# christianhbye/21cmVAE

Hardware: AMD Instinct MI355X
Metric: emulated signals/sec (batched predict) (higher is better)
Workload: dtype f16 (f32 accumulate)

## Files before the change

21cmvae_amd/csrc/api_forward.hip:

```cpp
#include "api_internal.h"

namespace v21 {
#define V21_DECL(a)                                                      \
  hipError_t launch_fused_##a##_F32(const FusedArgs&, hipStream_t);      \
  hipError_t launch_fused_##a##_F16x2sp(const FusedArgs&, hipStream_t);  \
  hipError_t launch_fused_##a##_BF16x2sp(const FusedArgs&, hipStream_t);
V21_ARCH_LIST(V21_DECL)
#undef V21_DECL
hipError_t launch_fused_S1_F16x2spClk(const FusedArgs&, hipStream_t);
hipError_t launch_fused_S1_BF16x2spClk(const FusedArgs&, hipStream_t);
}

typedef hipError_t (*fused_launcher)(const FusedArgs&, hipStream_t);
struct FusedEntry {
  int L;
  const int* dims;
  const int* act;
  fused_launcher fn[3];
};
#define V21_ENTRY(a) \
  {Arch##a::L, Arch##a::dims, Arch##a::act, {launch_fused_##a##_F32, launch_fused_##a##_F16x2sp, launch_fused_##a##_BF16x2sp}},
static const FusedEntry g_fused[] = {V21_ARCH_LIST(V21_ENTRY)};
#undef V21_ENTRY


static int fpi_of(int prec) { return prec == V21_PREC_F32 ? 8 : 16; }
static void stream_geometry(const v21_mlp* m, int prec, int* total, int* padded) {
  int f = 0;
  for (int l = 0; l < m->L; ++l) f += ((m->dims[l + 1] + 31) / 32) * ((m->dims[l] + fpi_of(prec) - 1) / fpi_of(prec) + 1);
  *total = f;
  *padded = (f + 7) / 8 * 8;
}

static int fused_id_of(int n_layers, const int* dims, const int* act) {
  for (size_t i = 0; i < sizeof(g_fused) / sizeof(g_fused[0]); ++i) {
    const FusedEntry& fe = g_fused[i];
    if (fe.L != n_layers) continue;
    bool same = true;
    for (int k = 0; k <= n_layers && same; ++k) same = fe.dims[k] == dims[k];
    for (int k = 0; k < n_layers && same; ++k) same = fe.act[k] == act[k];
    if (same) return (int)i;
// ... 72 lines not shown
  return V21_OK;
}
extern "C" int v21_mlp_destroy(v21_mlp* m) {
  if (!m) return V21_OK;
  hipSetDevice(m->ctx->device);
  hipStreamSynchronize(m->ctx->stream);
  delete m;
  return V21_OK;
}
extern "C" int v21_mlp_num_params(const v21_mlp* m, size_t* n) {
  if (!m || !n) return fail(V21_ERR_ARG, "null argument");
  *n = m->nparams;
  return V21_OK;
}
void invalidate_streams(v21_mlp* m) {
  for (int i = 0; i < 3; ++i) m->stream_ok[i] = false;
  for (int i = 0; i < 3; ++i) m->cfw_ok[i] = false;
  m->wpad_ok = false;
  m->wt_ok = false;
}

extern "C" int v21_mlp_set_weights(v21_mlp* m, const float* flat, size_t n) {
  if (!m || !flat) return fail(V21_ERR_ARG, "null argument");
  if (n != m->nparams) return fail(V21_ERR_ARG, "set_weights: got %zu floats, stack has %zu", n, m->nparams);
  CHK(use(m->ctx));
  HIPCHK(hipMemcpyAsync(m->d_w, flat, n * sizeof(float), hipMemcpyHostToDevice, m->ctx->stream));
  HIPCHK(hipStreamSynchronize(m->ctx->stream));
  invalidate_streams(m);
  return V21_OK;
}
extern "C" int v21_mlp_get_weights(v21_mlp* m, float* flat, size_t n) {
// ... 27 lines not shown
  if (t->n != m->dims[m->L] || !t->mean) return fail(V21_ERR_ARG, "output transform: n = %d, stack output = %d", t->n, m->dims[m->L]);
  CHK(m->d_mean.reserve((size_t)t->n));
  HIPCHK(hipMemcpyAsync(m->d_mean, t->mean, (size_t)t->n * sizeof(float), hipMemcpyHostToDevice, m->ctx->stream));
  HIPCHK(hipStreamSynchronize(m->ctx->stream));
  m->out_std = t->std;
  m->has_tout = true;
  return V21_OK;
}
extern "C" int v21_mlp_has_fused(const v21_mlp* m, int precision, int* yes) {
  if (!m || !yes) return fail(V21_ERR_ARG, "null argument");
  if (precision < 0 || precision > 2) return fail(V21_ERR_ARG, "precision %d unknown", precision);
  *yes = m->fused_id >= 0 ? 1 : 0;
  return V21_OK;
}

static int ensure_stream(v21_mlp* m, int prec) {
  if (m->stream_ok[prec]) return V21_OK;
  int total, padded;
  stream_geometry(m, prec, &total, &padded);
  Dev<unsigned char>& dst = m->d_stream[prec];
  CHK(dst.reserve((size_t)padded * 1024));
  PackArgs pa{};
  pa.w = m->d_w;
  pa.mean = m->has_tout ? m->d_mean : nullptr;
  pa.stream = dst;
  pa.L = m->L;
  pa.total = total;
  pa.padded = padded;
  pa.fpi = fpi_of(prec);
  pa.epi = prec == V21_PREC_F32 ? 4 : 8;
  pa.esize = prec == V21_PREC_F32 ? 4 : 2;
  pa.is_bf16 = prec == V21_PREC_BF16;
  int f = 0;
  for (int l = 0; l < m->L; ++l) {
    PackLayer& pl = pa.lt[l];
    pl.K = m->dims[l]; pl.N = m->dims[l + 1];
    pl.ks = (pl.K + pa.fpi - 1) / pa.fpi; pl.nt = (pl.N + 31) / 32;
    pl.w_off = m->w_off[l]; pl.b_off = m->b_off[l];
    pl.first = f;
    f += pl.nt * (pl.ks + 1);
  }
  hipLaunchKernelGGL(pack_stream_kernel, dim3((padded + 3) / 4), dim3(256), 0, m->ctx->stream, pa);
  HIPCHK(hipGetLastError());
  m->stream_ok[prec] = true;
  return V21_OK;
}

int mlp_fused_stream(v21_mlp* m, int prec, const unsigned char** stream) {
  CHK(ensure_stream(m, prec));
  *stream = m->d_stream[prec];
  return V21_OK;
}

template <class P, int EP>
static int launch_gemm(GemmArgs g, hipStream_t st) {
  if (g.M <= 0 || g.N <= 0) return V21_OK;
  dim3 grid((g.N + kBN - 1) / kBN, (g.M + kBM - 1) / kBM);
  const bool akc = g.sa_k == 1, bkc = g.sb_k == 1;
  if (!akc && g.sa_m != 1) return fail(V21_ERR_ARG, "gemm: A must be contiguous along m or k");
  if (!bkc && g.sb_n != 1) return fail(V21_ERR_ARG, "gemm: B must be contiguous along k or n");
  if (akc && bkc) hipLaunchKernelGGL((gemm_kernel<P, EP, true, true>), grid, dim3(256), 0, st, g);
  else if (akc) hipLaunchKernelGGL((gemm_kernel<P, EP, true, false>), grid, dim3(256), 0, st, g);
  else if (bkc) hipLaunchKernelGGL((gemm_kernel<P, EP, false, true>), grid, dim3(256), 0, st, g);
  else hipLaunchKernelGGL((gemm_kernel<P, EP, false, false>), grid, dim3(256), 0, st, g);
  HIPCHK(hipGetLastError());
  return V21_OK;
}
// ... 102 lines not shown
      (!(flags & V21_FWD_IN_TRANSFORM) || m->dims[0] <= 8)) {
    v21::JitKernel* k = jit_kernel(m, precision);
    if (force_jit && k) v21::jit_wait(k, -1);
    if (jit_ready(k)) jk = k;
    if (force_jit && !jk) {
      std::string why = "not eligible, or V21_JIT=0";
      if (k) v21::jit_state(k, &why);
      return fail(V21_ERR_UNSUPPORTED, "V21_FWD_FORCE_JIT: no run-time kernel for this stack: %s", why.c_str());
    }
  }
  q.jit = jk ? 2 : 0;
  int route = decide_forward(q);
  FusedArgs a{};
  hipError_t rt = hipSuccess;
  if (route == FWD_FUSED || route == FWD_FUSED_RT) {
    CHK(ensure_stream(m, precision));
    a.x = d_x; a.ldx = ldx; a.y = d_y; a.ldy = ldy; a.n_rows = n;
    a.stream = m->d_stream[precision];
    const bool tout = (flags & V21_FWD_OUT_TRANSFORM) != 0;
    a.out_std = tout ? m->out_std : 1.0f;
    a.out_mean_scale = tout ? 1.0f : 0.0f;
    a.in_transform = (flags & V21_FWD_IN_TRANSFORM) ? 1 : 0;
    if (a.in_transform) a.tin = m->tin;
#ifdef V21_FUSED_STAMP
    a.dbg = (unsigned long long*)(getenv("V21_FUSED_DBG_PTR") ? strtoull(getenv("V21_FUSED_DBG_PTR"), nullptr, 0) : 0ull);
#endif
  }
  if (route == FWD_FUSED_RT) {
    rt = v21::jit_launch(jk, m->ctx->device, a, m->ctx->stream);
    if (rt != hipSuccess) (void)hipGetLastError();
    if (rt != hipSuccess && !force_jit) { q.jit = 0; route = decide_forward(q); }
  }
  note_route(m, route);
// ... 270 lines not shown
```

21cmvae_amd/csrc/api_internal.h:

```cpp
#pragma once
#include <dlfcn.h>
#include <hip/hip_runtime.h>

#include <algorithm>
#include <climits>
#include <cmath>
#include <cstdarg>
#include <cstdio>
#include <cstdlib>
#include <cstring>
#include <functional>
#include <memory>
#include <string>
#include <vector>

#pragma GCC visibility push(default)
#include "../../include/v21.h"
#pragma GCC visibility pop
#include "archs.h"
#include "fused_fwd.h"
#include "jit.h"
#include "gemm.h"
#include "gemm_nt.h"
#include "train_kernels.h"
// ... 99 lines not shown
};

struct NuisRecord {
  std::vector<double> q, r, cd;
  std::vector<float> qf, proj;
};

struct v21_mlp {
  v21_ctx* ctx = nullptr;
  int L = 0;
  std::vector<int> dims, act;
  std::vector<long long> w_off, b_off;
  size_t nparams = 0;
  Dev<float> d_w;
  int fused_id = -1;
  Dev<unsigned char> d_stream[3];
  bool stream_ok[3] = {false, false, false};
  bool has_tin = false, has_tout = false;
  v21_affine_in tin{};
  float out_std = 1.f;
  Dev<float> d_mean;
  Dev<float> d_act[2];
  Dev<float> d_xs, d_ys;
  Dev<double> d_xs64;
  int maxdim = 0;
  bool wpad_ok = false;
  Dev<float> d_wt;
  std::vector<long long> wt_off;
  bool wt_ok = false;
  Dev<float> d_small[2];
  Dev<float> d_xpad;
  Dev<unsigned char> d_cfw[3], d_cbw[3];
// ... 234 lines not shown
```

21cmvae_amd/csrc/fused_fwd.h:

```cpp
#pragma once
#ifndef __HIPCC_RTC__
#include <hip/hip_runtime.h>
#endif

#include <type_traits>
#include <utility>

#include "../../include/v21_types.h"
#include "par_transform.h"

namespace v21 {

typedef float f32x16 __attribute__((ext_vector_type(16)));
typedef float f32x4 __attribute__((ext_vector_type(4)));
typedef _Float16 f16x8 __attribute__((ext_vector_type(8)));
typedef __bf16 bf16x8 __attribute__((ext_vector_type(8)));
typedef unsigned u32x4 __attribute__((ext_vector_type(4)));
typedef short i16x2 __attribute__((ext_vector_type(2)));
typedef float f32x2 __attribute__((ext_vector_type(2)));
typedef _Float16 f16x2 __attribute__((ext_vector_type(2)));
typedef __bf16 bf16x2 __attribute__((ext_vector_type(2)));

constexpr int kFragBytes = 1024;
constexpr int kWaves = 4;
// ... 30 lines not shown
  long long n_rows;
  const unsigned char* stream;
  float out_std;
  float out_mean_scale;
  int in_transform;
  v21_affine_in tin;
  unsigned long long* dbg;
};

struct PrecF16 {
  static constexpr int BLK = 24, RING = 4, WPS = 1, DEPTH = 2, WAVES = 4;
  using frag = f16x8;
  using elem = _Float16;
  static constexpr int FPI = 16, EPI = 8, CT = 2;
  static constexpr int WPI = 4;
  static __device__ __forceinline__ unsigned pack2(float a, float b) {
    f32x2 v = {a, b};
    return __builtin_bit_cast(unsigned, __builtin_convertvector(v, f16x2));
  }
  template <bool SWAP> static __device__ __forceinline__ f32x16 mfma(frag w, frag x, f32x16 c) {
    if constexpr (!SWAP) return __builtin_amdgcn_mfma_f32_32x32x16_f16(w, x, c, 0, 0, 0);
    else return __builtin_amdgcn_mfma_f32_32x32x16_f16(x, w, c, 0, 0, 0);
  }
};
struct PrecBF16 {
  static constexpr int BLK = 24, RING = 4, WPS = 1, DEPTH = 2, WAVES = 4;
  using frag = bf16x8;
  using elem = __bf16;
  static constexpr int FPI = 16, EPI = 8, CT = 2;
  static constexpr int WPI = 4;
  static __device__ __forceinline__ unsigned pack2(float a, float b) {
    f32x2 v = {a, b};
    return __builtin_bit_cast(unsigned, __builtin_convertvector(v, bf16x2));
  }
  template <bool SWAP> static __device__ __forceinline__ f32x16 mfma(frag w, frag x, f32x16 c) {
    if constexpr (!SWAP) return __builtin_amdgcn_mfma_f32_32x32x16_bf16(w, x, c, 0, 0, 0);
    else return __builtin_amdgcn_mfma_f32_32x32x16_bf16(x, w, c, 0, 0, 0);
  }
};
struct PrecF32 {
  static constexpr int BLK = 24, RING = 4, WPS = 1, DEPTH = 2, WAVES = 4;
  using frag = f32x4;
  using elem = float;
  static constexpr int FPI = 8, EPI = 4, CT = 1;
  static constexpr int WPI = 4;
// ... 11 lines not shown
struct PrecF16x2 : PrecF16 { static constexpr int CT = 1, BLK = 16, RING = 4, WPS = 2; };
struct PrecBF16x2 : PrecBF16 { static constexpr int CT = 1, BLK = 16, RING = 4, WPS = 2; };
#else
struct PrecF16x2 : PrecF16 { static constexpr int CT = 1, BLK = 16, RING = 5, WPS = 2; };
struct PrecBF16x2 : PrecBF16 { static constexpr int CT = 1, BLK = 16, RING = 5, WPS = 2; };
#endif

struct PrecF16x2sp : PrecF16x2 { static constexpr bool SPREAD_DMA = true; };
struct PrecBF16x2sp : PrecBF16x2 { static constexpr bool SPREAD_DMA = true; };
struct PrecF16x2spClk : PrecF16x2sp { static constexpr bool CLOCK_STAMPS = true; };
struct PrecBF16x2spClk : PrecBF16x2sp { static constexpr bool CLOCK_STAMPS = true; };
template <class P, class = void> struct clk_of { static constexpr bool value = false; };
template <class P> struct clk_of<P, std::void_t<decltype(P::CLOCK_STAMPS)>> { static constexpr bool value = P::CLOCK_STAMPS; };
template <class P, class = void> struct spread_of { static constexpr bool value = false; };
template <class P> struct spread_of<P, std::void_t<decltype(P::SPREAD_DMA)>> { static constexpr bool value = P::SPREAD_DMA; };

template <class Arch, class P> struct Geo {
  static constexpr int L = Arch::L;
  static constexpr int FPI = P::FPI;
  static constexpr int BLK = P::BLK, RING = P::RING, WAVES = P::WAVES;
  static constexpr int IPT = 16 / P::EPI;
  static constexpr int dim(int i) { return Arch::dims[i]; }
  static constexpr int act(int l) { return Arch::act[l]; }
  static constexpr int ks_of(int l) { return (dim(l) + FPI - 1) / FPI; }
  static constexpr int nt_of(int l) { return (dim(l + 1) + 31) / 32; }
  static constexpr int tile_base(int l, int nt) {
    int f = 0;
    for (int i = 0; i < l; ++i) f += nt_of(i) * (ks_of(i) + 1);
    return f + nt * (ks_of(l) + 1);
  }
// ... 44 lines not shown
  static constexpr int chunks_per_kstep(int G, int nchunks) {
    const int lim = spread_limit(G);
    return lim <= 0 ? nchunks : (nchunks + lim - 1) / lim;
  }
  static constexpr int stores_before_step(int S, int CT, int D) {
    int s = 0;
    const int l = L - 1, nch = CT * 8;
    for (int nt = 0; nt + 1 < nt_of(l); ++nt) {
      const int cpk = chunks_per_kstep(gtile(l, nt), nch);
      const int nb = tile_base(l, nt + 1);
      for (int c = 0; c < nch; ++c)
        if (nb + 1 + c / cpk + D < S) s += 2;
    }
    return s;
  }
};

template <int N> __device__ __forceinline__ void wait_vmcnt_barrier() {
  static_assert(N >= 0 && N <= 63, "vmcnt is 6 bits");
  asm volatile("s_waitcnt vmcnt(%0)\n\ts_barrier" ::"n"(N) : "memory");
}

__device__ __forceinline__ void glds16(const unsigned char* sbase, unsigned voff, unsigned lds_dst) {
  asm volatile("s_mov_b32 m0, %2\n\ts_nop 0\n\tglobal_load_lds_dwordx4 %0, %1"
               :
               : "v"(voff), "s"(sbase), "s"(lds_dst)
               : "memory");
}
__device__ __forceinline__ unsigned lds_addr(const void* p) {
  return (unsigned)(unsigned long long)(const __attribute__((address_space(3))) void*)p;
// ... 16 lines not shown

template <class G, int B, int I>
__device__ __forceinline__ void issue_piece(const unsigned char* gstream, unsigned char* smem,
                                            int wave, int lane) {
  if constexpr (B >= 0 && B < G::n_blocks()) {
    if constexpr (I < G::blk_glds(B)) {
      const unsigned char* g = gstream + (size_t)B * G::BLK * kFragBytes + I * G::WAVES * kFragBytes;
      const unsigned voff = wave * kFragBytes + lane * 16;
      const unsigned s = lds_addr(smem) + (B % G::RING) * G::BLK * kFragBytes + wave * kFragBytes +
                         I * G::WAVES * kFragBytes;
      glds16(g, voff, s);
    }
  }
}

template <class G, int CT, int D, int S, bool SPREAD>
__device__ __forceinline__ void ring_boundary(const unsigned char* gstream, unsigned char* smem,
                                              int wave, int lane, unsigned long long* g_dbg = nullptr) {
  constexpr int kBlkFrags = G::BLK, kRing = G::RING;
  if constexpr (S % kBlkFrags == 0 && S < G::padded()) {
    constexpr int B = S / kBlkFrags;
    constexpr int last_issued = (B + kRing - 3 > kRing - 1) ? B + kRing - 3 : kRing - 1;
    constexpr int GA = [] {
      int s = 0;
      for (int i = B + 1; i <= last_issued; ++i) s += G::blk_glds(i);
      return s;
    }();
    constexpr int S_issue = (B < kRing) ? 0 : (B - kRing + 2 + (SPREAD ? 1 : 0)) * kBlkFrags;
    constexpr int SA = G::stores_before_step(S, CT, D) - G::stores_before_step(S_issue, CT, D);
    constexpr int N = (GA + SA) > 63 ? 63 : (GA + SA);
#ifdef V21_FUSED_STAMP
    { unsigned long long t; asm volatile("s_memtime %0\n\ts_waitcnt lgkmcnt(0)" : "=s"(t)::"memory");
      ((unsigned long long*)(smem + G::RING * G::BLK * kFragBytes))[wave * 512 + 2 * B] = t; }
#endif
    wait_vmcnt_barrier<N>();
#ifdef V21_FUSED_STAMP
    { unsigned long long t; asm volatile("s_memtime %0\n\ts_waitcnt lgkmcnt(0)" : "=s"(t)::"memory");
      ((unsigned long long*)(smem + G::RING * G::BLK * kFragBytes))[wave * 512 + 2 * B + 1] = t; }
#endif
    if constexpr (B >= 2 && !SPREAD) issue_block<G, B + kRing - 2>(gstream, smem, wave, lane);
  }
}

template <class G, int F> __device__ __forceinline__ const unsigned char* frag_ptr(const unsigned char* smem, int lane) {
  constexpr int B = F / G::BLK;
// ... 10 lines not shown
  using frag = typename P::frag;
  using Item = typename G::Item;
  constexpr int L = G::L, CT = P::CT, EPI = P::EPI, FPI = P::FPI, IPT = G::IPT;
  constexpr int KSM = G::ks_max();
#ifndef V21_FUSED_D
#define V21_FUSED_D 2
#endif
#ifndef V21_FUSED_SPREAD
#define V21_FUSED_SPREAD 0
#endif
  constexpr int D = P::DEPTH;
  constexpr bool SPREAD = (V21_FUSED_SPREAD != 0) || spread_of<P>::value;
  constexpr int TOTAL = G::total();
  constexpr int NOUT = G::dim(L);
  constexpr int NCH = CT * 8;
  static_assert(G::act(L - 1) == 0, "output layer must be linear");
  static_assert(G::nt_of(L - 1) == 1 || G::ks_of(L - 1) > P::DEPTH, "output layer: too few k-steps per tile for the aux double buffer");
  static_assert(D <= kBlkFrags, "read-ahead must stay within one block");

  const int lane = threadIdx.x & 63;
  const int wave = __builtin_amdgcn_readfirstlane(threadIdx.x >> 6);
  const int r = lane & 31, h = lane >> 5;
  unsigned long long clk_t0 = 0, clk_r0 = 0;
  if constexpr (clk_of<P>::value) {
    asm volatile("s_memtime %0\n\ts_memrealtime %1\n\ts_waitcnt lgkmcnt(0)" : "=s"(clk_t0), "=s"(clk_r0)::"memory");
  }
  const long long wg_row0 = (long long)blockIdx.x * (kWaves * CT * 32);
  const long long row0 = wg_row0 + wave * (CT * 32);

  unsigned bufA[CT][KSM][4], bufB[CT][KSM][4];
// ... 43 lines not shown
    issue_block<G, decltype(b)::value>(a.stream, smem, wave, lane);
  });

  long long wg_rows = a.n_rows - wg_row0;
  if (wg_rows > kWaves * CT * 32) wg_rows = kWaves * CT * 32;
  if (wg_rows < 0) wg_rows = 0;
  const unsigned out_bytes = (unsigned)(wg_rows * a.ldy * 4);
  __amdgpu_buffer_rsrc_t orsrc =
      __builtin_amdgcn_make_buffer_rsrc((void*)(a.y + wg_row0 * a.ldy), 0, out_bytes, 0x00020000);
  const unsigned ldy_b = (unsigned)a.ldy * 4u;
  const unsigned ovoff = (unsigned)(wave * (CT * 32) + 4 * h) * ldy_b + (unsigned)r * 4u;

  frag q[D + 1];
  f32x16 auxb[2];
  f32x16 acc[2][CT];

  auto epilogue_chunk = [&](auto g_, auto c_) __attribute__((always_inline)) {
    constexpr int GT = decltype(g_)::value;
    constexpr int c = decltype(c_)::value;
    constexpr Item t = G::tile_at(GT);
    constexpr int l = t.l, nt = t.nt;
    constexpr int ct = c / 8, pr = c % 8;
    if constexpr (l < L - 1) {
      constexpr int item = IPT * nt + (2 * pr) / EPI, e0 = (2 * pr) % EPI;
      if constexpr (item < G::ks_of(l + 1)) {
        auto& out = (l & 1) ? bufA : bufB;
        const float x0 = acc[GT & 1][ct][2 * pr], x1 = acc[GT & 1][ct][2 * pr + 1];
        if constexpr (EPI == 8) {
          unsigned w = P::pack2(x0, x1);
          if constexpr (G::act(l) != 0) {
// ... 28 lines not shown
  };
  auto epilogue_range = [&](auto g_, auto lo_, auto hi_) __attribute__((always_inline)) {
    constexpr int LO = decltype(lo_)::value, HI = decltype(hi_)::value;
    static_for<(HI > LO ? HI - LO : 0)>([&](auto k) __attribute__((always_inline)) {
      epilogue_chunk(g_, std::integral_constant<int, LO + decltype(k)::value>{});
    });
  };
  auto operand = [&](auto& buf, int ct, int ks) __attribute__((always_inline)) {
    const u32x4 wds = {buf[ct][ks][0], buf[ct][ks][1], buf[ct][ks][2], buf[ct][ks][3]};
    return __builtin_bit_cast(frag, wds);
  };

  static_for<TOTAL + D>([&](auto s_) __attribute__((always_inline)) {
    constexpr int S = decltype(s_)::value;
    if constexpr (S < TOTAL) {
      ring_boundary<G, CT, D, S, SPREAD>(a.stream, smem, wave, lane, a.dbg);
      if constexpr (SPREAD && S / kBlkFrags >= 2) {
        constexpr int Bc = S / kBlkFrags, o = S % kBlkFrags;
#ifndef V21_SP_PHASE
#define V21_SP_PHASE 3
#endif
        if constexpr (o % G::WAVES == V21_SP_PHASE % G::WAVES)
          issue_piece<G, Bc + kRing - 2, o / G::WAVES>(a.stream, smem, wave, lane);
      }
      constexpr Item it = G::item_at(S);
      if constexpr (it.ks >= 0) {
        q[S % (D + 1)] = *(const frag*)frag_ptr<G, S>(smem, lane);
      } else {
        constexpr int GT = G::gtile(it.l, it.nt);
        const unsigned char* aux = frag_ptr<G, S>(smem, 0);
        if constexpr (it.l < L - 1) {
          const f32x4* bp = (const f32x4*)(aux + h * 64);
#pragma unroll
          for (int qd = 0; qd < 4; ++qd) {
            const f32x4 t = bp[qd];
            auxb[GT & 1][4 * qd + 0] = t[0]; auxb[GT & 1][4 * qd + 1] = t[1];
            auxb[GT & 1][4 * qd + 2] = t[2]; auxb[GT & 1][4 * qd + 3] = t[3];
          }
        } else {
          auxb[GT & 1][0] = ((const float*)aux)[r];
          auxb[GT & 1][1] = ((const float*)aux)[32 + r];
        }
      }
    }
    if constexpr (S >= D) {
      constexpr int C = S - D;
      constexpr Item it = G::item_at(C);
      if constexpr (it.ks >= 0) {
        constexpr int GT = G::gtile(it.l, it.nt);
        constexpr int GP = GT > 0 ? GT - 1 : 0;
        constexpr int CPK = G::chunks_per_kstep(GP, NCH);
        constexpr bool whole_first = (GT > 0) && (G::spread_limit(GP) == 0);
        if constexpr (whole_first && it.ks == 0) {
          epilogue_range(std::integral_constant<int, GP>{}, std::integral_constant<int, 0>{},
                         std::integral_constant<int, NCH>{});
        }
#ifdef V21_FUSED_STAMP
        if constexpr (it.ks == 0) {
          unsigned long long t; asm volatile("s_memtime %0\n\ts_waitcnt lgkmcnt(0)" : "=s"(t)::"memory");
          ((unsigned long long*)(smem + kFusedLds))[wave * 512 + 128 + GT] = t; }
#endif
        auto& in = (it.l & 1) ? bufB : bufA;
        const frag w = q[C % (D + 1)];
#pragma unroll
        for (int ct = 0; ct < CT; ++ct) {
          f32x16 c0;
          if constexpr (it.ks == 0) {
            if constexpr (it.l < L - 1) c0 = auxb[GT & 1];
            else
#pragma unroll
              for (int i = 0; i < 16; ++i) c0[i] = 0.f;
          } else {
            c0 = acc[GT & 1][ct];
          }
          acc[GT & 1][ct] = P::template mfma<(it.l == L - 1)>(w, operand(in, ct, it.ks), c0);
        }
        if constexpr (GT > 0 && !whole_first) {
          constexpr int lo = it.ks * CPK < NCH ? it.ks * CPK : NCH;
          constexpr int hi = (it.ks + 1) * CPK < NCH ? (it.ks + 1) * CPK : NCH;
          epilogue_range(std::integral_constant<int, GP>{}, std::integral_constant<int, lo>{},
                         std::integral_constant<int, hi>{});
        }
      }
    }
  });
  epilogue_range(std::integral_constant<int, G::n_tiles() - 1>{}, std::integral_constant<int, 0>{},
                 std::integral_constant<int, NCH>{});
  if constexpr (clk_of<P>::value) {
    unsigned long long t1, r1;
    unsigned xcc, hwid;
    asm volatile("s_memtime %0\n\ts_memrealtime %1\n\ts_getreg_b32 %2, hwreg(HW_REG_XCC_ID)\n\ts_getreg_b32 %3, hwreg(HW_REG_HW_ID)\n\ts_waitcnt lgkmcnt(0)"
                 : "=s"(t1), "=s"(r1), "=s"(xcc), "=s"(hwid)::"memory");
    if (a.dbg && wave == 0 && lane == 0) {
      unsigned long long* gd = a.dbg + (size_t)blockIdx.x * 5;
      gd[0] = clk_t0; gd[1] = clk_r0; gd[2] = t1; gd[3] = r1; gd[4] = (unsigned long long)(xcc & 0xF) | ((unsigned long long)hwid << 8);
    }
  }
#ifdef V21_FUSED_STAMP
  if (a.dbg) {
    unsigned long long t; asm volatile("s_memtime %0\n\ts_waitcnt lgkmcnt(0)" : "=s"(t)::"memory");
    unsigned long long* sd = (unsigned long long*)(smem + kFusedLds) + wave * 512;
    sd[127] = t;
// ... 10 lines not shown
```

21cmvae_amd/csrc/jit.hip:

```cpp
#include "jit.h"
#include "fused_train16.h"

#include <dlfcn.h>
#include <signal.h>
#include <spawn.h>
#include <sys/stat.h>
#include <sys/wait.h>
#include <unistd.h>

#include <atomic>
#include <chrono>
#include <condition_variable>
#include <cstdio>
#include <cstdlib>
#include <cerrno>
#include <cstring>
#include <map>
#include <mutex>
#include <thread>
#include <vector>

namespace v21 {
namespace {

// ... 79 lines not shown
    return base_prec(prec) == 1 ? Launch{kTrain16RowsPerWg, 64 * PrecF16t16::WAVES, fused_train16_lds<PrecF16t16>()}
                                : Launch{kTrain16RowsPerWg, 64 * PrecBF16t16::WAVES, fused_train16_lds<PrecBF16t16>()};
  if (prec == 0) return launch_of<PrecF32>();
  if (prec == 1) return wide ? launch_of<PrecF16>() : launch_of<PrecF16x2sp>();
  return wide ? launch_of<PrecBF16>() : launch_of<PrecBF16x2sp>();
}

unsigned long long fnv1a(const void* p, size_t n, unsigned long long h = 1469598103934665603ull) {
  const unsigned char* b = (const unsigned char*)p;
  for (size_t i = 0; i < n; ++i) { h ^= b[i]; h *= 1099511628211ull; }
  return h;
}

const char* kOptions[] = {"--offload-arch=gfx950", "-std=c++20", "-O3", "-ffp-contract=off", "-mllvm", "-amdgpu-mfma-vgpr-form=1"};
constexpr int kNumOptions = sizeof(kOptions) / sizeof(kOptions[0]);

std::string lib_dir() {
  Dl_info info{};
  if (dladdr((const void*)&fnv1a, &info) && info.dli_fname) {
    std::string p = info.dli_fname;
    const size_t s = p.rfind('/');
    return s == std::string::npos ? "." : p.substr(0, s);
  }
  return ".";
}
void mkdirs(const std::string& d, mode_t leaf = 0755) {
  for (size_t i = 1; i <= d.size(); ++i)
    if (i == d.size() || d[i] == '/') mkdir(d.substr(0, i).c_str(), i == d.size() ? leaf : 0755);
}
bool private_dir(const std::string& d) {
// ... 123 lines not shown
  return src;
}
constexpr int kCacheFormat = 2;
int toolchain_version() {
  if (const char* e = getenv("V21_JIT_TOOLCHAIN")) return atoi(e);
  static const int cached = [] {
    int v = 0;
    if (hipRuntimeGetVersion(&v) != hipSuccess) { (void)hipGetLastError(); v = 0; }
    return v;
  }();
  return cached;
}
std::string file_name(const JitKernel& k) {
  unsigned long long h = is_train(k.prec) ? fnv1a(kTrainSrc, sizeof(kTrainSrc)) : fnv1a(kFusedSrc, sizeof(kFusedSrc));
  for (int i = 0; i < kNumOptions; ++i) h = fnv1a(kOptions[i], strlen(kOptions[i]), h);
  h = fnv1a(k.spec.data(), k.spec.size(), h);
  const int meta[3] = {kCacheFormat, toolchain_version(), HIP_VERSION};
  h = fnv1a(meta, sizeof meta, h);
  char buf[32];
  snprintf(buf, sizeof buf, "%016llx", h);
  return "fused_" + k.spec + "_" + buf + ".v21k";
}

int compile(const JitKernel& k, std::string& sym, std::vector<char>& code, std::string& why) {
  if (!load_rtc(&why)) return -1;
  const std::string src = make_source(k);
  const std::string expr = std::string(is_train(k.prec) ? "v21::fused_train16<v21::ArchRT, v21::" : "v21::fused_fwd<v21::ArchRT, v21::") +
                           prec_type(k.prec, k.wide) + ">";
  rtc_prog prog = nullptr;
  int r = g_rtc.CreateProgram(&prog, src.c_str(), "v21_fused_rt.hip", 0, nullptr, nullptr);
  if (r != 0) { why = "hiprtcCreateProgram failed"; return -1; }
  r = g_rtc.AddNameExpression(prog, expr.c_str());
  std::vector<const char*> opts(kOptions, kOptions + kNumOptions);
  std::string depth_opt;
  if (is_train(k.prec) && train_depth(k.L, k.dims) != V21_TRAIN16_DEPTH) {
    depth_opt = "-DV21_TRAIN16_DEPTH=" + std::to_string(train_depth(k.L, k.dims));
    opts.push_back(depth_opt.c_str());
  }
  if (r == 0) r = g_rtc.CompileProgram(prog, (int)opts.size(), opts.data());
  if (r != 0) {
    size_t n = 0;
    g_rtc.GetProgramLogSize(prog, &n);
    std::string log(n, '\0');
    if (n) g_rtc.GetProgramLog(prog, log.data());
    if (log.size() > 1500) log.resize(1500);
    why = std::string("hiprtc: ") + (g_rtc.GetErrorString ? g_rtc.GetErrorString(r) : "?") + ": " + log;
    g_rtc.DestroyProgram(&prog);
    return -1;
  }
// ... 228 lines not shown
```

21cmvae_amd/csrc/train_kernels.h:

```cpp
#pragma once
#include <hip/hip_runtime.h>

#include "../../include/v21.h"
#include "par_transform.h"
#include "chain_types.h"

namespace v21 {

static __global__ void step_tick_kernel(int* cur) { *cur += 1; }

template <bool WRITE_GRAD>
__global__ void loss_grad_kernel(const float* __restrict__ p, long long ldp,
                                 const float* __restrict__ y, long long ldy,
                                 const float* __restrict__ w, float* __restrict__ dz,
                                 long long lddz, float* __restrict__ rowloss, int n, int d,
                                 float scale, const float* __restrict__ extra) {
  const int row = blockIdx.x * (blockDim.x >> 6) + (threadIdx.x >> 6);
  const int lane = threadIdx.x & 63;
  if (row >= n) return;
  const float wi = w[row];
  const float gs = scale * wi;
  const float* pr = p + (long long)row * ldp;
  const float* yr = y + (long long)row * ldy;
  float s = 0.f;
// ... 439 lines not shown
  if (i >= n * ld16) return;
  const long long r = i / ld16; const int c = (int)(i - r * ld16);
  const float v = c < din ? x[r * din + c] : 0.f;
  if (is_bf16) { const __bf16 h = (__bf16)v; out[i] = __builtin_bit_cast(unsigned short, h); }
  else { const _Float16 h = (_Float16)v; out[i] = __builtin_bit_cast(unsigned short, h); }
}
struct PackLayer { int K, N, ks, nt; long long w_off, b_off; int first; int flags; };
struct PackArgs {
  const float* w;
  const float* mean;
  unsigned char* stream;
  int L, total, padded, fpi, epi, esize;
  int is_bf16;
  int all_hidden;
  int fmt16;
  PackLayer lt[32];
};
static __global__ void pack_stream_kernel(const PackArgs a) {
  const int F = blockIdx.x * (blockDim.x >> 6) + (threadIdx.x >> 6);
  const int lane = threadIdx.x & 63;
  if (F >= a.padded) return;
  unsigned char* dst = a.stream + (size_t)F * 1024;
  if (F >= a.total) {
    ((float4*)dst)[lane] = make_float4(0.f, 0.f, 0.f, 0.f);
    return;
  }
  int l = 0;
  while (l + 1 < a.L && F >= a.lt[l + 1].first) ++l;
  const PackLayer L = a.lt[l];
  const int rel = F - L.first, tl = L.ks + 1;
  const int nt = rel / tl, ks = rel % tl - 1;
  if (a.fmt16) {
// ... 18 lines not shown
    return;
  }
  const int r = lane & 31, h = lane >> 5;
  if (ks < 0) {
    float out[4] = {0.f, 0.f, 0.f, 0.f};
    for (int q = 0; q < 4; ++q) {
      const int idx = lane * 4 + q;
      float v = 0.f;
      if (l < a.L - 1 || a.all_hidden) {
        if (idx < 32 && !(L.flags & 2)) {
          const int hh = idx >> 4, reg = idx & 15;
          const int n = 32 * nt + (reg & 3) + 8 * (reg >> 2) + 4 * hh;
          if (n < L.N) v = a.w[L.b_off + n];
        }
      } else {
        if (idx < 32) { const int n = 32 * nt + idx; if (n < L.N) v = a.w[L.b_off + n]; }
        else if (idx < 64) { const int n = 32 * nt + idx - 32; if (n < L.N && a.mean) v = a.mean[n]; }
      }
      out[q] = v;
    }
    ((float4*)dst)[lane] = make_float4(out[0], out[1], out[2], out[3]);
    return;
  }
  const int n = 32 * nt + r;
  for (int e = 0; e < a.epi; ++e) {
    const int f = a.fpi * ks + 8 * (e >> 2) + 4 * h + (e & 3);
    float v = 0.f;
    if (f < L.K && n < L.N) v = (L.flags & 1) ? a.w[L.w_off + (long long)n * L.K + f] : a.w[L.w_off + (long long)f * L.N + n];
    if (a.esize == 4) ((float*)dst)[lane * 4 + e] = v;
    else if (a.is_bf16) ((__bf16*)dst)[lane * 8 + e] = (__bf16)v;
    else ((_Float16*)dst)[lane * 8 + e] = (_Float16)v;
  }
}

}
```

__graft_entry__.py:

```python
import importlib
import json
import os
import subprocess
import sys

ROOT = os.path.dirname(os.path.abspath(__file__))
if ROOT not in sys.path:
    sys.path.insert(0, ROOT)


def build():
    csrc = os.path.join(ROOT, "21cmvae_amd", "csrc")
    jobs = str(min(8, os.cpu_count() or 1))
    subprocess.run(["make", "-C", csrc, "-j", jobs], check=True)
    ora = os.path.join(ROOT, "oracle")
    if os.path.exists(os.path.join(ora, "Makefile")):
        subprocess.run(["make", "-C", ora], check=True)
    native = importlib.import_module("21cmvae_amd._native")
    native.load_library()
    importlib.import_module("21cmvae_amd")
    prebuild_kernels()


PREBUILT_STACKS = [
    ([7, 64, 128, 451], [1, 1, 0]),
    ([7, 32, 128, 256, 451], [1, 1, 1, 0]),
    ([7, 288, 352, 288, 224, 9], [1, 1, 1, 1, 0]),
    ([451, 352, 9], [1, 0]),
    ([9, 500, 512, 33], [1, 1, 0]),
    ([7, 352, 352, 352, 224, 451], [1, 1, 1, 1, 0]),
    ([7, 352, 352, 352, 352, 352, 352, 9], [1, 1, 1, 1, 1, 1, 0]),
]


PREBUILT_TRAIN_STACKS = [
    ([7, 64, 128, 451], [1, 1, 0]),
    ([451, 128, 4, 32, 128, 451], [1, 0, 1, 1, 0]),
]


_PREBUILD_CHILD = """
import importlib, json, sys
sys.path.insert(0, sys.argv[1])
native = importlib.import_module("21cmvae_amd._native")
dims, act, prec = json.loads(sys.argv[2])
if prec.startswith("train_"):
# ... 128 lines not shown
```

Baseline: 1.134 billion.

## Group output tiles into 16-byte stores with permuted weight packing

For the 16-bit fused forward kernels, the output layer now keeps accumulators for groups of four 32-column tiles. The packed weight stream permutes the output columns so that each lane can write four adjacent outputs with one 128-bit buffer store instead of four 32-bit stores. Store issue is spread across the next job's k-steps, and the ring wait counts are recomputed from a new schedule model. The change costs more accumulator registers and a second cached stream layout per precision, and it also adds -fno-slp-vectorize to the JIT forward compile.

```diff
diff --git a/21cmvae_amd/csrc/api_forward.hip b/21cmvae_amd/csrc/api_forward.hip
--- a/21cmvae_amd/csrc/api_forward.hip
+++ b/21cmvae_amd/csrc/api_forward.hip
@@ -25,6 +25,9 @@
 
 
 static int fpi_of(int prec) { return prec == V21_PREC_F32 ? 8 : 16; }
+static_assert(v21::out_group_of<PrecF16x2sp>::value == v21::out_group_of<PrecBF16x2sp>::value && v21::out_group_of<PrecF16x2spClk>::value == v21::out_group_of<PrecF16x2sp>::value &&
+              v21::out_group_of<PrecBF16x2spClk>::value == v21::out_group_of<PrecF16x2sp>::value, "one output layout for the 16-bit forward kernels");
+static int out_group_for(int prec) { return prec == V21_PREC_F32 ? v21::out_group_of<PrecF32>::value : v21::out_group_of<PrecF16x2sp>::value; }
 static void stream_geometry(const v21_mlp* m, int prec, int* total, int* padded) {
   int f = 0;
   for (int l = 0; l < m->L; ++l) f += ((m->dims[l + 1] + 31) / 32) * ((m->dims[l] + fpi_of(prec) - 1) / fpi_of(prec) + 1);
@@ -127,7 +130,7 @@
   return V21_OK;
 }
 void invalidate_streams(v21_mlp* m) {
-  for (int i = 0; i < 3; ++i) m->stream_ok[i] = false;
+  for (int i = 0; i < 3; ++i) m->stream_ok[0][i] = m->stream_ok[1][i] = false;
   for (int i = 0; i < 3; ++i) m->cfw_ok[i] = false;
   m->wpad_ok = false;
   m->wt_ok = false;
@@ -185,11 +188,13 @@
   return V21_OK;
 }
 
-static int ensure_stream(v21_mlp* m, int prec) {
-  if (m->stream_ok[prec]) return V21_OK;
+static int ensure_stream(v21_mlp* m, int prec, int out_group, const unsigned char** stream) {
+  const int lay = out_group > 1 ? 1 : 0;
+  *stream = nullptr;
+  if (m->stream_ok[lay][prec]) { *stream = m->d_stream[lay][prec]; return V21_OK; }
   int total, padded;
   stream_geometry(m, prec, &total, &padded);
-  Dev<unsigned char>& dst = m->d_stream[prec];
+  Dev<unsigned char>& dst = m->d_stream[lay][prec];
   CHK(dst.reserve((size_t)padded * 1024));
   PackArgs pa{};
   pa.w = m->d_w;
@@ -202,6 +207,7 @@
   pa.epi = prec == V21_PREC_F32 ? 4 : 8;
   pa.esize = prec == V21_PREC_F32 ? 4 : 2;
   pa.is_bf16 = prec == V21_PREC_BF16;
+  pa.out_group = out_group;
   int f = 0;
   for (int l = 0; l < m->L; ++l) {
     PackLayer& pl = pa.lt[l];
@@ -213,15 +219,12 @@
   }
   hipLaunchKernelGGL(pack_stream_kernel, dim3((padded + 3) / 4), dim3(256), 0, m->ctx->stream, pa);
   HIPCHK(hipGetLastError());
-  m->stream_ok[prec] = true;
-  return V21_OK;
-}
-
-int mlp_fused_stream(v21_mlp* m, int prec, const unsigned char** stream) {
-  CHK(ensure_stream(m, prec));
-  *stream = m->d_stream[prec];
-  return V21_OK;
-}
+  m->stream_ok[lay][prec] = true;
+  *stream = dst;
+  return V21_OK;
+}
+
+int mlp_fused_stream(v21_mlp* m, int prec, const unsigned char** stream) { return ensure_stream(m, prec, 1, stream); }
 
 template <class P, int EP>
 static int launch_gemm(GemmArgs g, hipStream_t st) {
@@ -354,9 +357,8 @@
   FusedArgs a{};
   hipError_t rt = hipSuccess;
   if (route == FWD_FUSED || route == FWD_FUSED_RT) {
-    CHK(ensure_stream(m, precision));
+    CHK(ensure_stream(m, precision, out_group_for(precision), &a.stream));
     a.x = d_x; a.ldx = ldx; a.y = d_y; a.ldy = ldy; a.n_rows = n;
-    a.stream = m->d_stream[precision];
     const bool tout = (flags & V21_FWD_OUT_TRANSFORM) != 0;
     a.out_std = tout ? m->out_std : 1.0f;
     a.out_mean_scale = tout ? 1.0f : 0.0f;
diff --git a/21cmvae_amd/csrc/api_internal.h b/21cmvae_amd/csrc/api_internal.h
--- a/21cmvae_amd/csrc/api_internal.h
+++ b/21cmvae_amd/csrc/api_internal.h
@@ -137,8 +137,8 @@
   size_t nparams = 0;
   Dev<float> d_w;
   int fused_id = -1;
-  Dev<unsigned char> d_stream[3];
-  bool stream_ok[3] = {false, false, false};
+  Dev<unsigned char> d_stream[2][3];
+  bool stream_ok[2][3] = {};
   bool has_tin = false, has_tout = false;
   v21_affine_in tin{};
   float out_std = 1.f;
diff --git a/21cmvae_amd/csrc/fused_fwd.h b/21cmvae_amd/csrc/fused_fwd.h
--- a/21cmvae_amd/csrc/fused_fwd.h
+++ b/21cmvae_amd/csrc/fused_fwd.h
@@ -68,6 +68,7 @@
   using elem = _Float16;
   static constexpr int FPI = 16, EPI = 8, CT = 2;
   static constexpr int WPI = 4;
+  static constexpr int OUT_GROUP = 4;
   static __device__ __forceinline__ unsigned pack2(float a, float b) {
     f32x2 v = {a, b};
     return __builtin_bit_cast(unsigned, __builtin_convertvector(v, f16x2));
@@ -83,6 +84,7 @@
   using elem = __bf16;
   static constexpr int FPI = 16, EPI = 8, CT = 2;
   static constexpr int WPI = 4;
+  static constexpr int OUT_GROUP = 4;
   static __device__ __forceinline__ unsigned pack2(float a, float b) {
     f32x2 v = {a, b};
     return __builtin_bit_cast(unsigned, __builtin_convertvector(v, bf16x2));
@@ -124,6 +126,11 @@
 template <class P> struct clk_of<P, std::void_t<decltype(P::CLOCK_STAMPS)>> { static constexpr bool value = P::CLOCK_STAMPS; };
 template <class P, class = void> struct spread_of { static constexpr bool value = false; };
 template <class P> struct spread_of<P, std::void_t<decltype(P::SPREAD_DMA)>> { static constexpr bool value = P::SPREAD_DMA; };
+template <class P, class = void> struct out_group_of { static constexpr int value = 1; };
+template <class P> struct out_group_of<P, std::void_t<decltype(P::OUT_GROUP)>> { static constexpr int value = P::OUT_GROUP; };
+#ifndef V21_SP_PHASE
+#define V21_SP_PHASE 3
+#endif
 
 template <class Arch, class P> struct Geo {
   static constexpr int L = Arch::L;
@@ -198,6 +205,61 @@
     }
     return s;
   }
+
+  static constexpr int OG = out_group_of<P>::value;
+  static constexpr int out_groups() { return OG > 1 ? dim(L) / (32 * OG) : 0; }
+  static constexpr int out_jobs() { return out_groups() + nt_of(L - 1) - OG * out_groups(); }
+  struct OutJob { int nt0, tiles, units, stores_per_unit; };
+  static constexpr OutJob out_job(int j) {
+    const int ng = out_groups();
+    if (j < ng) return OutJob{OG * j, OG, P::CT * 16, 1};
+    return OutJob{OG * ng + (j - ng), 1, P::CT * 8, 2};
+  }
+  static constexpr int out_job_of(int nt) {
+    const int ng = out_groups();
+    return nt < OG * ng ? nt / OG : ng + nt - OG * ng;
+  }
+  static constexpr int out_slot(int nt) {
+    const int ng = out_groups();
+    return nt < OG * ng ? ((nt / OG) & 1) * OG + nt % OG : (ng & 1) * OG + (nt - OG * ng);
+  }
+  struct OutUnits { int job, lo, hi; };
+  static constexpr OutUnits out_units_at(int nt, int ks) {
+    const int j = out_job_of(nt);
+    if (j == 0) return OutUnits{-1, 0, 0};
+    const OutJob me = out_job(j), pv = out_job(j - 1);
+    const int nk = me.tiles * ks_of(L - 1), k = (nt - me.nt0) * ks_of(L - 1) + ks;
+    return OutUnits{j - 1, (k * pv.units + nk - 1) / nk, ((k + 1) * pv.units + nk - 1) / nk};
+  }
+  static constexpr int dma_at(int S, bool spread) {
+    if (S < 0 || S >= total()) return 0;
+    const int B = S / BLK, o = S % BLK;
+    if (B < 2) return 0;
+    if (!spread) return o == 0 ? blk_glds(B + RING - 2) : 0;
+    return (o % WAVES == V21_SP_PHASE % WAVES && o / WAVES < blk_glds(B + RING - 2)) ? 1 : 0;
+  }
+  static constexpr int stores_at(int S, int D) {
+    if (S < D || S - D >= total()) return 0;
+    const Item it = item_at(S - D);
+    if (it.l != L - 1 || it.ks < 0) return 0;
+    const OutUnits u = out_units_at(it.nt, it.ks);
+    return u.job < 0 ? 0 : (u.hi - u.lo) * out_job(u.job).stores_per_unit;
+  }
+  static constexpr int last_piece_step(int B, bool spread) {
+    return (B - RING + 2) * BLK + (spread ? (blk_glds(B) - 1) * WAVES + V21_SP_PHASE % WAVES : 0);
+  }
+  static constexpr int vm_after_block(int B, int D, bool spread) {
+    int n = 0, s0 = 0;
+    if (B < RING) {
+      for (int i = B + 1; i < RING; ++i) n += blk_glds(i);
+    } else {
+      s0 = last_piece_step(B, spread);
+      n = stores_at(s0, D);
+      ++s0;
+    }
+    for (int s = s0; s < B * BLK; ++s) n += dma_at(s, spread) + stores_at(s, D);
+    return n;
+  }
 };
 
 template <int N> __device__ __forceinline__ void wait_vmcnt_barrier() {
@@ -244,7 +306,7 @@
   }
 }
 
-template <class G, int CT, int D, int S, bool SPREAD>
+template <class G, int CT, int D, int S, bool SPREAD, bool GROUPED = false>
 __device__ __forceinline__ void ring_boundary(const unsigned char* gstream, unsigned char* smem,
                                               int wave, int lane, unsigned long long* g_dbg = nullptr) {
   constexpr int kBlkFrags = G::BLK, kRing = G::RING;
@@ -257,8 +319,17 @@
       return s;
     }();
     constexpr int S_issue = (B < kRing) ? 0 : (B - kRing + 2 + (SPREAD ? 1 : 0)) * kBlkFrags;
-    constexpr int SA = G::stores_before_step(S, CT, D) - G::stores_before_step(S_issue, CT, D);
+    constexpr int SA = [] {
+      if constexpr (GROUPED) {
+        int s = 0;
+        for (int i = (B < kRing ? 0 : G::last_piece_step(B, SPREAD)); i < S; ++i) s += G::stores_at(i, D);
+        return s;
+      } else {
+        return G::stores_before_step(S, CT, D) - G::stores_before_step(S_issue, CT, D);
+      }
+    }();
     constexpr int N = (GA + SA) > 63 ? 63 : (GA + SA);
+    static_assert(!GROUPED || N <= G::vm_after_block(B, D, SPREAD), "ring wait counts more operations than were issued behind block B");
 #ifdef V21_FUSED_STAMP
     { unsigned long long t; asm volatile("s_memtime %0\n\ts_waitcnt lgkmcnt(0)" : "=s"(t)::"memory");
       ((unsigned long long*)(smem + G::RING * G::BLK * kFragBytes))[wave * 512 + 2 * B] = t; }
@@ -299,6 +370,9 @@
   constexpr int TOTAL = G::total();
   constexpr int NOUT = G::dim(L);
   constexpr int NCH = CT * 8;
+  constexpr int OG = G::OG;
+  constexpr bool GROUPED = OG > 1;
+  static_assert(OG == 1 || (OG == 4 && EPI == 8), "grouped output layer: four tiles per 16-byte store, 16-bit operands");
   static_assert(G::act(L - 1) == 0, "output layer must be linear");
   static_assert(G::nt_of(L - 1) == 1 || G::ks_of(L - 1) > P::DEPTH, "output layer: too few k-steps per tile for the aux double buffer");
   static_assert(D <= kBlkFrags, "read-ahead must stay within one block");
@@ -372,6 +446,41 @@
   frag q[D + 1];
   f32x16 auxb[2];
   f32x16 acc[2][CT];
+  constexpr int NSLOT = GROUPED ? 2 * OG : 1;
+  f32x16 oacc[NSLOT][CT];
+  float okc[NSLOT], oaux[2];
+  const unsigned gvoff = (unsigned)(wave * (CT * 32) + 4 * h) * ldy_b + (unsigned)r * 16u;
+  auto out_unit = [&](auto j_, auto u_) __attribute__((always_inline)) {
+    constexpr int J = decltype(j_)::value, u = decltype(u_)::value;
+    constexpr typename G::OutJob jb = G::out_job(J);
+    if constexpr (J < G::out_groups()) {
+      constexpr int ct = u / 16, i = u % 16;
+      f32x4 y;
+      static_for<4>([&](auto t_) __attribute__((always_inline)) {
+        constexpr int t = decltype(t_)::value, sl = G::out_slot(jb.nt0 + t);
+        y[t] = __builtin_fmaf(oacc[sl][ct][i], a.out_std, okc[sl]);
+      });
+      const unsigned soff = (unsigned)(ct * 32 + (i & 3) + 8 * (i >> 2)) * ldy_b + (unsigned)(32 * OG * J) * 4u;
+      __builtin_amdgcn_raw_buffer_store_b128(__builtin_bit_cast(u32x4, y), orsrc, gvoff, soff, 0);
+    } else {
+      constexpr int ct = u / 8, pr = u % 8, nt = jb.nt0, sl = G::out_slot(nt);
+      unsigned voff = ovoff + (unsigned)(32 * nt) * 4u;
+      if (32 * nt + r >= NOUT) voff = 0xFFFFFFF0u;
+#pragma unroll
+      for (int w = 0; w < 2; ++w) {
+        const int i = 2 * pr + w;
+        const unsigned soff = (unsigned)(ct * 32 + (i & 3) + 8 * (i >> 2)) * ldy_b;
+        const float y = __builtin_fmaf(oacc[sl][ct][i], a.out_std, okc[sl]);
+        __builtin_amdgcn_raw_buffer_store_b32(__builtin_bit_cast(unsigned, y), orsrc, voff, soff, 0);
+      }
+    }
+  };
+  auto out_units = [&](auto j_, auto lo_, auto hi_) __attribute__((always_inline)) {
+    constexpr int LO = decltype(lo_)::value, HI = decltype(hi_)::value;
+    static_for<(HI > LO ? HI - LO : 0)>([&](auto k) __attribute__((always_inline)) {
+      out_unit(j_, std::integral_constant<int, LO + decltype(k)::value>{});
+    });
+  };
 
   auto epilogue_chunk = [&](auto g_, auto c_) __attribute__((always_inline)) {
     constexpr int GT = decltype(g_)::value;
@@ -430,12 +539,11 @@
   static_for<TOTAL + D>([&](auto s_) __attribute__((always_inline)) {
     constexpr int S = decltype(s_)::value;
     if constexpr (S < TOTAL) {
-      ring_boundary<G, CT, D, S, SPREAD>(a.stream, smem, wave, lane, a.dbg);
+      ring_boundary<G, CT, D, S, SPREAD, GROUPED>(a.stream, smem, wave, lane, a.dbg);
       if constexpr (SPREAD && S / kBlkFrags >= 2) {
         constexpr int Bc = S / kBlkFrags, o = S % kBlkFrags;
-#ifndef V21_SP_PHASE
-#define V21_SP_PHASE 3
-#endif
+        static_assert(G::dma_at(S, true) == ((o % G::WAVES == V21_SP_PHASE % G::WAVES && o / G::WAVES < G::blk_glds(Bc + kRing - 2)) ? 1 : 0),
+                      "Geo::dma_at describes this schedule");
         if constexpr (o % G::WAVES == V21_SP_PHASE % G::WAVES)
           issue_piece<G, Bc + kRing - 2, o / G::WAVES>(a.stream, smem, wave, lane);
       }
@@ -453,6 +561,9 @@
             auxb[GT & 1][4 * qd + 0] = t[0]; auxb[GT & 1][4 * qd + 1] = t[1];
             auxb[GT & 1][4 * qd + 2] = t[2]; auxb[GT & 1][4 * qd + 3] = t[3];
           }
+        } else if constexpr (GROUPED) {
+          oaux[0] = ((const float*)aux)[r];
+          oaux[1] = ((const float*)aux)[32 + r];
         } else {
           auxb[GT & 1][0] = ((const float*)aux)[r];
           auxb[GT & 1][1] = ((const float*)aux)[32 + r];
@@ -467,7 +578,10 @@
         constexpr int GP = GT > 0 ? GT - 1 : 0;
         constexpr int CPK = G::chunks_per_kstep(GP, NCH);
         constexpr bool whole_first = (GT > 0) && (G::spread_limit(GP) == 0);
-        if constexpr (whole_first && it.ks == 0) {
+        constexpr bool OUTG = GROUPED && it.l == L - 1;
+        constexpr bool prev_out = OUTG && it.nt > 0;
+        constexpr int SL = OUTG ? G::out_slot(it.nt) : 0;
+        if constexpr (!prev_out && whole_first && it.ks == 0) {
           epilogue_range(std::integral_constant<int, GP>{}, std::integral_constant<int, 0>{},
                          std::integral_constant<int, NCH>{});
         }
@@ -487,11 +601,19 @@
 #pragma unroll
               for (int i = 0; i < 16; ++i) c0[i] = 0.f;
           } else {
-            c0 = acc[GT & 1][ct];
+            if constexpr (OUTG) c0 = oacc[SL][ct];
+            else c0 = acc[GT & 1][ct];
           }
-          acc[GT & 1][ct] = P::template mfma<(it.l == L - 1)>(w, operand(in, ct, it.ks), c0);
+          if constexpr (OUTG) oacc[SL][ct] = P::template mfma<true>(w, operand(in, ct, it.ks), c0);
+          else acc[GT & 1][ct] = P::template mfma<(it.l == L - 1)>(w, operand(in, ct, it.ks), c0);
         }
-        if constexpr (GT > 0 && !whole_first) {
+        if constexpr (OUTG && it.ks == 0) okc[SL] = __builtin_fmaf(oaux[0], a.out_std, oaux[1] * a.out_mean_scale);
+        if constexpr (prev_out) {
+          constexpr typename G::OutUnits un = G::out_units_at(it.nt, it.ks);
+          static_assert(G::stores_at(S, D) == (un.job < 0 ? 0 : (un.hi - un.lo) * G::out_job(un.job < 0 ? 0 : un.job).stores_per_unit), "Geo::stores_at describes this schedule");
+          if constexpr (un.job >= 0)
+            out_units(std::integral_constant<int, (un.job < 0 ? 0 : un.job)>{}, std::integral_constant<int, un.lo>{}, std::integral_constant<int, un.hi>{});
+        } else if constexpr (GT > 0 && !whole_first) {
           constexpr int lo = it.ks * CPK < NCH ? it.ks * CPK : NCH;
           constexpr int hi = (it.ks + 1) * CPK < NCH ? (it.ks + 1) * CPK : NCH;
           epilogue_range(std::integral_constant<int, GP>{}, std::integral_constant<int, lo>{},
@@ -500,8 +622,13 @@
       }
     }
   });
-  epilogue_range(std::integral_constant<int, G::n_tiles() - 1>{}, std::integral_constant<int, 0>{},
-                 std::integral_constant<int, NCH>{});
+  if constexpr (GROUPED) {
+    constexpr int J = G::out_jobs() - 1;
+    out_units(std::integral_constant<int, J>{}, std::integral_constant<int, 0>{}, std::integral_constant<int, G::out_job(J).units>{});
+  } else {
+    epilogue_range(std::integral_constant<int, G::n_tiles() - 1>{}, std::integral_constant<int, 0>{},
+                   std::integral_constant<int, NCH>{});
+  }
   if constexpr (clk_of<P>::value) {
     unsigned long long t1, r1;
     unsigned xcc, hwid;
diff --git a/21cmvae_amd/csrc/jit.hip b/21cmvae_amd/csrc/jit.hip
--- a/21cmvae_amd/csrc/jit.hip
+++ b/21cmvae_amd/csrc/jit.hip
@@ -117,6 +117,7 @@
 
 const char* kOptions[] = {"--offload-arch=gfx950", "-std=c++20", "-O3", "-ffp-contract=off", "-mllvm", "-amdgpu-mfma-vgpr-form=1"};
 constexpr int kNumOptions = sizeof(kOptions) / sizeof(kOptions[0]);
+const char* kFwdOption = "-fno-slp-vectorize";
 
 std::string lib_dir() {
   Dl_info info{};
@@ -270,6 +271,7 @@
 std::string file_name(const JitKernel& k) {
   unsigned long long h = is_train(k.prec) ? fnv1a(kTrainSrc, sizeof(kTrainSrc)) : fnv1a(kFusedSrc, sizeof(kFusedSrc));
   for (int i = 0; i < kNumOptions; ++i) h = fnv1a(kOptions[i], strlen(kOptions[i]), h);
+  if (!is_train(k.prec)) h = fnv1a(kFwdOption, strlen(kFwdOption), h);
   h = fnv1a(k.spec.data(), k.spec.size(), h);
   const int meta[3] = {kCacheFormat, toolchain_version(), HIP_VERSION};
   h = fnv1a(meta, sizeof meta, h);
@@ -289,6 +291,7 @@
   r = g_rtc.AddNameExpression(prog, expr.c_str());
   std::vector<const char*> opts(kOptions, kOptions + kNumOptions);
   std::string depth_opt;
+  if (!is_train(k.prec)) opts.push_back(kFwdOption);
   if (is_train(k.prec) && train_depth(k.L, k.dims) != V21_TRAIN16_DEPTH) {
     depth_opt = "-DV21_TRAIN16_DEPTH=" + std::to_string(train_depth(k.L, k.dims));
     opts.push_back(depth_opt.c_str());
diff --git a/21cmvae_amd/csrc/train_kernels.h b/21cmvae_amd/csrc/train_kernels.h
--- a/21cmvae_amd/csrc/train_kernels.h
+++ b/21cmvae_amd/csrc/train_kernels.h
@@ -477,8 +477,13 @@
   int is_bf16;
   int all_hidden;
   int fmt16;
+  int out_group;
   PackLayer lt[32];
 };
+static __device__ __forceinline__ int out_column(int nt, int r, int N, int og) {
+  if (og > 1 && 32 * og * (nt / og + 1) <= N) return 32 * og * (nt / og) + og * r + nt % og;
+  return 32 * nt + r;
+}
 static __global__ void pack_stream_kernel(const PackArgs a) {
   const int F = blockIdx.x * (blockDim.x >> 6) + (threadIdx.x >> 6);
   const int lane = threadIdx.x & 63;
@@ -527,15 +532,15 @@
           if (n < L.N) v = a.w[L.b_off + n];
         }
       } else {
-        if (idx < 32) { const int n = 32 * nt + idx; if (n < L.N) v = a.w[L.b_off + n]; }
-        else if (idx < 64) { const int n = 32 * nt + idx - 32; if (n < L.N && a.mean) v = a.mean[n]; }
+        if (idx < 32) { const int n = out_column(nt, idx, L.N, a.out_group); if (n < L.N) v = a.w[L.b_off + n]; }
+        else if (idx < 64) { const int n = out_column(nt, idx - 32, L.N, a.out_group); if (n < L.N && a.mean) v = a.mean[n]; }
       }
       out[q] = v;
     }
     ((float4*)dst)[lane] = make_float4(out[0], out[1], out[2], out[3]);
     return;
   }
-  const int n = 32 * nt + r;
+  const int n = (l == a.L - 1 && !a.all_hidden) ? out_column(nt, r, L.N, a.out_group) : 32 * nt + r;
   for (int e = 0; e < a.epi; ++e) {
     const int f = a.fpi * ks + 8 * (e >> 2) + 4 * h + (e & 3);
     float v = 0.f;
diff --git a/__graft_entry__.py b/__graft_entry__.py
--- a/__graft_entry__.py
+++ b/__graft_entry__.py
@@ -30,6 +30,7 @@
     ([9, 500, 512, 33], [1, 1, 0]),
     ([7, 352, 352, 352, 224, 451], [1, 1, 1, 1, 0]),
     ([7, 352, 352, 352, 352, 352, 352, 9], [1, 1, 1, 1, 1, 1, 0]),
+    ([7, 48, 100], [1, 0]), ([7, 48, 128], [1, 0]), ([7, 48, 129], [1, 0]), ([7, 48, 259], [1, 0]), ([7, 48, 451], [1, 0]),
 ]
 
 
```

New measurement: 1.115 billion. 0.983x the previous value.
